# Graph-COM/SUREL_Plus

Measured on AMD Instinct MI355X. Metric: query-pairs/sec (sample+SpJoin), higher is better.
Workload: dtype int32; 1 GPU; cit2-like LP: N=2,927,963 avg-deg 20.7 power-law graph, M=200, --num_steps 4 (m=3 hops); ranks_seen=1, distinct_devices=1, rng=philox

## Files before the change

surel_plus_amd/csrc/sjoin.hip:

```cpp
#include "sjoin_f64pair.hpp"

namespace subgacc {


template <bool F64, int KV, typename Val>
__device__ __forceinline__ void emit_rows(const JoinArgs &a, int lane, const int32_t *own_ids, const Val *own_val,
                                          int64_t na, const int32_t *pids, const Val *pval, int nb, int64_t t0,
                                          int64_t o, int64_t segj, int k, int k2, uint32_t magic) {
    const int64_t t = t0 + lane;
    const bool live = t < na;
    int32_t id = 0;
    Val va = 0;
    if (live) {
        id = own_ids[t];
        va = own_val[t];
    }
    int lo = 0, hi = live ? nb : 0;
    SJ_HOOK_SEARCH_RANGE(lo, hi);
    while (lo < hi) {
        const int mid = (lo + hi) >> 1;
        if (pids[mid] < id) lo = mid + 1;
        else hi = mid;
    }
    const bool hit = live && lo < nb && pids[lo] == id;
// ... 65 lines not shown
        ra = jj < half ? src : tgt, rb = jj < half ? tgt : src;
        int64_t sb, sn;
        join_row(a, src, sb, sn);
        if (sn <= a.star_cap) return;
        if (lane == 0) atomicOr(&a.flags[1], 2);
    } else
        ra = a.own[j], rb = join_partner(a, j);
    join_row(a, ra, ab, na);
    join_row(a, rb, bb, nb64);
    if (nb64 > (STAGE ? (int64_t)a.max_len : (int64_t)0x7FFFFFFF)) {
        if (lane == 0) atomicOr(&a.flags[3], 1);
        return;
    }
    const int nb = (int)nb64;
    const Val *data = (const Val *)a.data;
    if (STAGE) {
        for (int r = lane; r < nb; r += kJoinThreads) {
            pids[r] = a.indices[bb + r];
            pval[r] = data[bb + r];
        }
        __syncthreads();
    } else {
        pids = const_cast<int32_t *>(a.indices + bb);
        pval = const_cast<Val *>(data + bb);
    }
    const int64_t o = a.seg[j];
    const int k = a.k, k2 = 2 * k;
    const uint32_t magic = k2 > 0 ? ((1u << 20) + (uint32_t)k2 - 1u) / (uint32_t)k2 : 0u;
    for (int64_t t0 = 0; t0 < na; t0 += kWave)
        emit_rows<F64, KV, Val>(a, lane, a.indices + ab, data + ab, na, pids, pval, nb, t0, o, j, k, k2, magic);
}


template <int KV, int NT, bool K64, bool TAB = false>
__global__ __launch_bounds__(NT) void sjoin_keypair_kernel(const JoinArgs a, uint32_t pb, uint32_t pairs) {
    extern __shared__ __align__(16) unsigned char lds_raw[];
    static_assert(!(K64 && TAB), "a table row number is 32 bits");
    using Key = typename std::conditional<K64, unsigned long long, uint32_t>::type;
    constexpr int NW = NT / kWave;
    const bool xl = TAB && a.slot_id != nullptr;
    auto sfptr = [&](Key v) -> Key {
        if (!TAB) return v;
        return xl ? (Key)(a.slot_id[(int32_t)v] + 1) : (Key)((int32_t)v + a.val_add);
    };
    const int ML = a.max_len;
    Key *valT = (Key *)lds_raw;
    Key *pk = valT + ML;
    int32_t *idsT = (int32_t *)(pk + ML);
    const int kc = KV > 0 ? KV : a.k, w = 2 * kc;
    const int tid = threadIdx.x, lane = tid & (kWave - 1);
    const int wave = __builtin_amdgcn_readfirstlane(tid / kWave);
    const size_t stage_off = ((size_t)ML * (2 * sizeof(Key) + 4) + 15) & ~(size_t)15;
    float *stage = (float *)(lds_raw + stage_off) + wave * (kWave * w + 4);

    SJ_HOOK_PAIR_ENTRY();
    if (a.sized_here && (a.flags[3] & 64)) return;
    const uint32_t wg = (uint32_t)(blockIdx.x & (kXcds - 1)) * (gridDim.x / kXcds) + (blockIdx.x / kXcds);
    uint32_t p = wg, part = 0;
    if (a.split > 1) {
        p = wg / (uint32_t)a.split;
        part = wg - p * (uint32_t)a.split;
    }
    if (p >= pairs) return;
    uint32_t blk = 0, off = p;
    if (pb != pairs) {
        blk = p / pb;
        off = p - blk * pb;
// ... 139 lines not shown
        }
#pragma unroll
        for (int u = 0; u < kRegTrips; ++u) {
            sgot[u] = 0;
            if (u < trips) {
                const int32_t f = idsT[b[u]];
                const Key g = valT[b[u]];
                const bool hit = (wave + u * NW) * kWave + lane < ns && n == 1 && f == sid[u];
                if (hit) pk[b[u]] = skey[u], sgot[u] = g;
            }
        }
    }
    for (int c = wave + kRegTrips * NW; c < chunksS; c += NW) {
        const int t0 = c * kWave;
        const bool live = t0 + lane < ns;
        int32_t id = 0;
        Key key = 0;
        if (live) {
            id = stream_load(&a.indices[sb + t0 + lane]);
            key = sfptr(stream_load(&keys[sb + t0 + lane]));
        }
        int bx = 0, n = nt;
        SJ_HOOK_SEARCH_RANGE(bx, n);
        while (n > 1) {
            const int h = n >> 1;
            bx = idsT[bx + h] <= id ? bx + h : bx;
            n -= h;
        }
        const int32_t f = idsT[bx];
        const Key g = valT[bx];
        const bool hit = live && n == 1 && f == id;
        if (hit) pk[bx] = key;
        if (whole || (uint32_t)(c / NW) % (uint32_t)a.split == part)
            emit_key_span<KV, K64, TAB, Key>(a, lane, live, key, hit ? g : (Key)0, ns - t0 < kWave ? ns - t0 : kWave, oS + t0, jS, kc, q, stage);
    }
    __syncthreads();
#pragma unroll
    for (int u = 0; u < kRegTrips; ++u) {
        const int c = wave + u * NW, t0 = c * kWave;
        if (c < chunksS && (whole || (uint32_t)u % (uint32_t)a.split == part))
            emit_key_span<KV, K64, TAB, Key>(a, lane, t0 + lane < ns, skey[u], sgot[u], ns - t0 < kWave ? ns - t0 : kWave, oS + t0, jS, kc, q, stage);
    }
    const int rot = (NW - chunksS % NW) % NW;
    for (int c = (wave + rot) % NW + (int)part * NW; c < chunksT; c += a.split * NW) {
        const int t0 = c * kWave;
        const bool live = t0 + lane < nt;
        const int i = live ? t0 + lane : t0;
        emit_key_span<KV, K64, TAB, Key>(a, lane, live, valT[i], pk[i], nt - t0 < kWave ? nt - t0 : kWave, oT + t0, jT, kc, q, stage);
    }
}


template <int NT>
__global__ __launch_bounds__(NT) void sjoin_f64pair_kernel(const JoinArgs a, uint32_t pb, uint32_t pairs) {
    extern __shared__ __align__(16) unsigned char lds_raw[];
    constexpr int NW = NT / kWave;
    const int ML = a.max_len;
    double *valT = (double *)lds_raw;
    double *pv = valT + ML;
    int32_t *idsT = (int32_t *)(pv + ML);
    const int tid = threadIdx.x;
    const int wave = __builtin_amdgcn_readfirstlane(tid / kWave);

    SJ_HOOK_PAIR_ENTRY();
    if (a.sized_here && (a.flags[3] & 64)) return;
    F64Pair p;
    float2 *xz = reinterpret_cast<float2 *>(a.out_xz);
    int64_t *segid = a.out_segid;
    int32_t *flags = a.flags;
    const auto span_s = [xz, segid, &p](int t, bool emit, double v, double got) {
        if (emit) {
            float2 o;
            o.x = (float)v, o.y = (float)((got + 1.0) - 1.0);
            stream_store(xz + p.oS + t, o);
            if (segid) __builtin_nontemporal_store(p.jS, segid + p.oS + t);
        }
    };
    if (!f64pair_stage<NT, true>(a, pb, pairs, ML, valT, pv, idsT, p, span_s, [flags, tid]() {
            if (tid == 0) atomicOr(&flags[3], 1);
        }))
        return;
    __syncthreads();
    const int chunksS = (p.ns + kWave - 1) / kWave, chunksT = (p.nt + kWave - 1) / kWave;
    const int rot = (NW - chunksS % NW) % NW;
    for (int c = (wave + rot) % NW + (int)p.part * NW; c < chunksT; c += a.split * NW) {
        const int t = c * kWave + (tid & (kWave - 1));
        if (t < p.nt) {
            float2 o;
            o.x = (float)valT[t], o.y = (float)((pv[t] + 1.0) - 1.0);
            stream_store(xz + p.oT + t, o);
            if (a.out_segid) __builtin_nontemporal_store(p.jT, a.out_segid + p.oT + t);
        }
    }
}

template <int KV, int NT, int MODE>
__global__ __launch_bounds__(NT) void sjoin_star_kernel(const JoinArgs a, uint32_t P, uint32_t K, uint32_t chunk, uint32_t chunks) {
    extern __shared__ __align__(16) unsigned char lds_raw[];
    constexpr bool F64 = MODE == 2, TAB = MODE == 1;
    using Val = typename std::conditional<F64, double, uint32_t>::type;
    constexpr int NW = NT / kWave;
    const int cap = a.star_cap;
    Val *valA = (Val *)lds_raw;
    Val *pa = valA + cap;
    int32_t *idsA = (int32_t *)(pa + cap);
    const int kc = F64 ? 1 : (KV > 0 ? KV : a.k), w = 2 * kc;
    const int tid = threadIdx.x, lane = tid & (kWave - 1);
    const int wave = __builtin_amdgcn_readfirstlane(tid / kWave);
    const size_t stage_off = ((size_t)cap * (2 * sizeof(Val) + 4) + 15) & ~(size_t)15;
    float *stage = (float *)(lds_raw + stage_off) + wave * (kWave * w + 4);

    if (a.sized_here && (a.flags[3] & 64)) return;
    if (blockIdx.x == 0 && tid == 0) atomicOr(&a.flags[1], 1);
    const uint32_t wg = (uint32_t)(blockIdx.x & (kXcds - 1)) * (gridDim.x / kXcds) + (blockIdx.x / kXcds);
    const uint32_t p = wg / chunks, part = wg - p * chunks;
    if (p >= P) return;
    const uint32_t t_beg = part * chunk, t_end = t_beg + chunk < K ? t_beg + chunk : K;
    if (t_beg >= t_end) return;
    int64_t ab, na64;
    join_row(a, a.own[p], ab, na64);
    if (na64 > cap) {
        if (na64 > a.max_len && tid == 0) atomicOr(&a.flags[3], 1);
        return;
    }
    const int na = (int)na64;
    const Val *vals = (const Val *)a.data;
    for (int r = tid; r < na; r += NT) {
        idsA[r] = a.indices[ab + r];
        valA[r] = vals[ab + r];
// ... 6 lines not shown
    const int64_t half = (int64_t)P * K;
    __syncthreads();
    for (uint32_t t = t_beg; t < t_end; ++t) {
        const int64_t j = (int64_t)p * K + t, j2 = half + j;
        int64_t bb, nb64;
        join_row(a, a.partner[j], bb, nb64);
        const int nb = (int)nb64;
        const int64_t oA = a.seg[j], oB = a.seg[j2];
        const int chunksB = (nb + kWave - 1) / kWave;
        for (int c = wave; c < chunksB; c += NW) {
            const int t0 = c * kWave;
            const bool live = t0 + lane < nb;
            int32_t id = 0;
            Val v = 0;
            if (live) {
                id = stream_load(&a.indices[bb + t0 + lane]);
                v = stream_load(&vals[bb + t0 + lane]);
            }
            int bx;
            const bool hit = sorted_find(idsA, na, id, live, bx);
            Val g = 0;
            if (hit) {
                pa[bx] = v;
                g = valA[bx];
            }
            if constexpr (F64) {
                if (live) {
                    float2 o;
                    o.x = (float)v, o.y = (float)((g + 1.0) - 1.0);
                    stream_store(xz + oB + t0 + lane, o);
                    if (a.out_segid) __builtin_nontemporal_store(j2, a.out_segid + oB + t0 + lane);
                }
            } else
                emit_key_span<KV, false, TAB, uint32_t>(a, lane, live, v, g, nb - t0 < kWave ? nb - t0 : kWave, oB + t0, j2, kc, q, stage);
        }
        __syncthreads();
        const int rot = (NW - chunksB % NW) % NW;
        for (int c = (wave + rot) % NW; c < chunksA; c += NW) {
            const int t0 = c * kWave;
            const bool live = t0 + lane < na;
            const int i = live ? t0 + lane : t0;
            const Val v = valA[i], g = pa[i];
            if (live) pa[i] = 0;
            if constexpr (F64) {
                if (live) {
                    float2 o;
                    o.x = (float)v, o.y = (float)((g + 1.0) - 1.0);
                    stream_store(xz + oA + i, o);
                    if (a.out_segid) __builtin_nontemporal_store(j, a.out_segid + oA + i);
                }
            } else
                emit_key_span<KV, false, TAB, uint32_t>(a, lane, live, v, g, na - t0 < kWave ? na - t0 : kWave, oA + t0, j, kc, q, stage);
        }
        __syncthreads();
    }
}

}

using namespace subgacc;


static int launch_table_pairs(JoinArgs &a, int64_t S, int64_t pair_block, bool vec4, void *stream, const char *who) {
    const int k = a.out_xz ? a.k : 1;
    const size_t lds = (size_t)a.max_len * 12 + key_stage_bytes(kPairEmit / kWave, k);
    SG_REQUIRE(lds <= (size_t)kLdsBytes, SUBGACC_ERR_LDS, "%s: rows of %d members do not fit LDS", who, (int)a.max_len);
    a.split = pair_split(S / 2);
    int64_t grid;
    if (int rc = grid_of(S / 2 * a.split, who, grid)) return rc;
    void (*kernel)(JoinArgs, uint32_t, uint32_t);
    if (vec4) kernel = sjoin_keypair_kernel<4, kPairEmit, false, true>;
    else if (a.out_xz && a.k == 3) kernel = sjoin_keypair_kernel<3, kPairEmit, false, true>;
    else if (a.out_xz && a.k == 5) kernel = sjoin_keypair_kernel<5, kPairEmit, false, true>;
    else kernel = sjoin_keypair_kernel<0, kPairEmit, false, true>;
    return launch(kernel, grid, kPairEmit, lds, (hipStream_t)stream, a, (uint32_t)pair_block, (uint32_t)(S / 2));
}

static int key_args(JoinArgs &a, int32_t num_walks, int32_t num_steps, const char *who, bool wide) {
    const int shift = subgacc_key_shift(num_walks, num_steps);
    if (shift < 0) return shift;
    SG_REQUIRE(num_steps * shift + 1 <= (wide ? 63 : 31) && num_steps + 1 <= 16, SUBGACC_ERR_KEYWIDTH,
               "%s: LP keys of %d steps x %d bits do not fit %d bits", who, num_steps, shift, wide ? 64 : 32);
    a.k = num_steps + 1;
    a.key_M = num_walks, a.key_m = num_steps, a.key_shift = shift;
    return SUBGACC_OK;
}

static int launch_key_join(JoinArgs &a, int32_t num_walks, int32_t num_steps, int64_t S, int64_t pair_block, void *stream,
                           const char *who, bool wide = false) {
    const int rc = key_args(a, num_walks, num_steps, who, wide);
    if (rc != SUBGACC_OK) return rc;
    const int nt = (a.max_len > 512 && pair_split(S / 2) == 1 && (a.k == 4 || (wide && a.k == 5))) ? 256 : kPairEmit;
    const size_t lds = (size_t)a.max_len * (wide ? 20 : 12) + key_stage_bytes(nt / kWave, a.k);
    SG_REQUIRE(lds <= (size_t)kLdsBytes, SUBGACC_ERR_LDS, "%s: rows of %d members do not fit LDS", who, (int)a.max_len);
    a.split = pair_split(S / 2);
    int64_t grid;
    if (int rc = grid_of(S / 2 * a.split, who, grid)) return rc;
    void (*kernel)(JoinArgs, uint32_t, uint32_t);
    int threads = kPairEmit;
    if (wide) {
        if (a.k == 5 && nt == 256) kernel = sjoin_keypair_kernel<5, 256, true>, threads = 256;
        else if (a.k == 5) kernel = sjoin_keypair_kernel<5, kPairEmit, true>;
        else kernel = sjoin_keypair_kernel<0, kPairEmit, true>;
    } else if (a.k == 4 && nt == 256) kernel = sjoin_keypair_kernel<4, 256, false>, threads = 256;
    else if (a.k == 4) kernel = sjoin_keypair_kernel<4, kPairEmit, false>;
    else if (a.k == 3) kernel = sjoin_keypair_kernel<3, kPairEmit, false>;
    else if (a.k == 5) kernel = sjoin_keypair_kernel<5, kPairEmit, false>;
    else kernel = sjoin_keypair_kernel<0, kPairEmit, false>;
    return launch(kernel, grid, threads, lds, (hipStream_t)stream, a, (uint32_t)pair_block, (uint32_t)(S / 2));
}

static int launch_f64_pairs(JoinArgs &a, int64_t S, int64_t pair_block, void *stream) {
    const size_t flds = (size_t)a.max_len * 20 + 16;
    SG_REQUIRE(flds <= (size_t)kLdsBytes, SUBGACC_ERR_LDS, "sjoin_fill: float rows of %d members do not fit LDS", (int)a.max_len);
    a.split = pair_split(S / 2);
    int64_t grid;
    if (int rc = grid_of(S / 2 * a.split, "sjoin_fill", grid)) return rc;
    const uint32_t pairs = (uint32_t)(S / 2), pb32 = (uint32_t)pair_block;
    hipStream_t s = (hipStream_t)stream;
    if (a.max_len <= 2 * kWave) return launch(sjoin_f64pair_kernel<kWave>, grid, kWave, flds, s, a, pb32, pairs);
    return launch(sjoin_f64pair_kernel<kPairEmit>, grid, kPairEmit, flds, s, a, pb32, pairs);
}

static int launch_segments(JoinArgs &a, bool f64, bool vec4, void *stream) {
    size_t lds = (size_t)a.max_len * (f64 ? 12 : 8);
    const bool staged = lds <= (size_t)kLdsBytes;
    if (!staged) lds = 0;
    int64_t grid;
    if (int rc = grid_of(a.S, "sjoin_fill", grid)) return rc;
    void (*kernel)(JoinArgs);
    if (!staged) {
        if (f64) kernel = sjoin_fill_kernel<true, 0, false>;
        else if (vec4) kernel = sjoin_fill_kernel<false, 4, false>;
        else kernel = sjoin_fill_kernel<false, 0, false>;
    } else if (f64) kernel = sjoin_fill_kernel<true, 0>;
    else if (vec4) kernel = sjoin_fill_kernel<false, 4>;
    else kernel = sjoin_fill_kernel<false, 0>;
    return launch(kernel, grid, kJoinThreads, lds, (hipStream_t)stream, a);
}

#ifndef SJ_STAR_GROUPS
#define SJ_STAR_GROUPS 8192
#endif
constexpr int64_t kStarGroups = SJ_STAR_GROUPS;
static int launch_star(JoinArgs &a, int mode, bool vec4, bool packed, int64_t K, void *stream) {
    const int64_t S = a.S, P = S / (2 * K);
    SG_REQUIRE(S / 2 < (1ll << 31), SUBGACC_ERR_BADARG, "sjoin_fill_v2: the star option (OPT_STAR) joins fewer than 2^31 pairs, not %lld", (long long)(S / 2));
    const bool f64 = mode == 2;
    const int nt = f64 && a.max_len <= 2 * kWave ? kWave : kPairEmit;
    const size_t per = f64 ? 20 : 12, stage = f64 ? 16 : key_stage_bytes(nt / kWave, a.k);
    const size_t room = (size_t)kLdsBytes - stage - 16;
    int64_t cap = a.max_len;
    if ((size_t)cap * per > room) cap = (int64_t)(room / per);
    SG_REQUIRE(cap == a.max_len || (packed && mode != 0), SUBGACC_ERR_LDS, "sjoin_fill_v2: rows of %d members do not fit LDS",
               (int)a.max_len);
    a.star_k = K, a.star_cap = (int32_t)cap;
    int64_t chunks = ceil_div(kStarGroups, P);
    if (chunks > K) chunks = K;
    const int64_t chunk = ceil_div(K, chunks);
    chunks = ceil_div(K, chunk);
    int64_t grid;
    if (int rc = grid_of(P * chunks, "sjoin_fill_v2", grid)) return rc;
    const size_t lds = (((size_t)cap * per + 15) & ~(size_t)15) + stage;
    void (*kernel)(JoinArgs, uint32_t, uint32_t, uint32_t, uint32_t);
    if (f64 && nt == kWave) kernel = sjoin_star_kernel<0, kWave, 2>;
    else if (f64) kernel = sjoin_star_kernel<0, kPairEmit, 2>;
    else if (mode == 1 && vec4) kernel = sjoin_star_kernel<4, kPairEmit, 1>;
    else if (mode == 1 && a.k == 3) kernel = sjoin_star_kernel<3, kPairEmit, 1>;
    else if (mode == 1 && a.k == 5) kernel = sjoin_star_kernel<5, kPairEmit, 1>;
    else if (mode == 1) kernel = sjoin_star_kernel<0, kPairEmit, 1>;
    else if (a.k == 4) kernel = sjoin_star_kernel<4, kPairEmit, 0>;
    else if (a.k == 3) kernel = sjoin_star_kernel<3, kPairEmit, 0>;
    else if (a.k == 5) kernel = sjoin_star_kernel<5, kPairEmit, 0>;
    else kernel = sjoin_star_kernel<0, kPairEmit, 0>;
    if (int rc = launch(kernel, grid, nt, lds, (hipStream_t)stream, a, (uint32_t)P, (uint32_t)K, (uint32_t)chunk, (uint32_t)chunks))
        return rc;
    if (cap < a.max_len) return launch_segments(a, f64, vec4, stream);
    return SUBGACC_OK;
}

extern "C" int subgacc_sjoin_fill_v2(const subgacc_join_desc *d, void *stream) {
    RowLayout layout;
    if (int rc = decode_desc("sjoin_fill_v2", d, false, layout)) return rc;
    const bool packed = layout == RowLayout::Packed, strided = layout == RowLayout::Strided;
    SG_REQUIRE((d->options & ~(SUBGACC_JOIN_OPT_SIZES | SUBGACC_JOIN_OPT_STAR)) == 0, SUBGACC_ERR_BADARG,
               "sjoin_fill_v2: unknown option bits %d", (int)d->options);
    SG_REQUIRE(d->form >= SUBGACC_JOIN_ROWS && d->form <= SUBGACC_JOIN_PAIRS, SUBGACC_ERR_BADARG, "sjoin_fill_v2: unknown form %d", (int)d->form);
    SG_REQUIRE(d->payload_kind >= SUBGACC_JOIN_SFPTR && d->payload_kind <= SUBGACC_JOIN_KEY64, SUBGACC_ERR_BADARG,
               "sjoin_fill_v2: unknown payload kind %d", (int)d->payload_kind);
    const int kind = d->payload_kind;
    const bool f64 = kind == SUBGACC_JOIN_F64, keyed = kind == SUBGACC_JOIN_KEY32 || kind == SUBGACC_JOIN_KEY64;
    const bool sized = (d->options & SUBGACC_JOIN_OPT_SIZES) != 0;
    const bool sizes_only = sized && !d->out_xz && !d->out_idx;
    const bool star = (d->options & SUBGACC_JOIN_OPT_STAR) != 0;
    const int64_t *seg = sized ? d->out_seg : d->seg;
    const int64_t S = d->S, pb = d->pair_block;
    SG_REQUIRE(!sized || d->form == SUBGACC_JOIN_ROWS, SUBGACC_ERR_BADARG, "sjoin_fill_v2: OPT_SIZES goes with the row form");
    if (star) {
        SG_REQUIRE(d->form == SUBGACC_JOIN_ROWS, SUBGACC_ERR_BADARG, "sjoin_fill_v2: the star option (OPT_STAR) goes with the row form (not the count or pair form)");
        SG_REQUIRE(!strided, SUBGACC_ERR_BADARG, "sjoin_fill_v2: the star option (OPT_STAR) joins packed or headed rows, not strided rows");
        SG_REQUIRE(kind != SUBGACC_JOIN_KEY64, SUBGACC_ERR_BADARG, "sjoin_fill_v2: the star option (OPT_STAR) does not join 64-bit keys (KEY64)");
        SG_REQUIRE(pb > 0, SUBGACC_ERR_BADARG, "sjoin_fill_v2: the star option (OPT_STAR) needs pair_block = K > 0 targets per source (pair_block = %lld)",
                   (long long)pb);
// ... 81 lines not shown
```

surel_plus_amd/csrc/sjoin.hpp:

```cpp
#pragma once
#include <cstdlib>
#include <type_traits>
#include "common.hpp"

namespace subgacc {

constexpr int kJoinThreads = 64;
constexpr int kPairThreads = 256;
#ifndef SJ_PAIR_THREADS
#define SJ_PAIR_THREADS 128
#endif
constexpr int kPairEmit = SJ_PAIR_THREADS;
constexpr int kMeanThreads = kPairEmit;
constexpr int kMeanCap = 1024;

struct JoinArgs {
    const int64_t *indptr;
    const int32_t *indices;
    const void *data;
    const int64_t *own, *partner, *seg;
    int64_t S;
    int64_t n_rows;
    const float *table;
    int64_t table_rows;
// ... 116 lines not shown
            sid[u] = 0, sval[u] = 0;
            if (r < ns) sid[u] = stream_load(&a.indices[sb + r]), sval[u] = stream_load(&data[sb + r]);
        }
    }
    __device__ __forceinline__ void get(const JoinArgs &a, int64_t sb, int r0, int r, int32_t &id, int32_t &value) const {
        const int u = r0 / kPairThreads;
        const int32_t i0 = sid[0], i1 = sid[1], v0 = sval[0], v1 = sval[1];
        if (u < kTrips) {
            id = u == 0 ? i0 : i1;
            value = u == 0 ? v0 : v1;
        } else {
            id = stream_load(&a.indices[sb + r]);
            value = stream_load(&((const int32_t *)a.data)[sb + r]);
        }
    }
};

struct KeyQuot {
    float fm, rcp;
    bool divide;
};
__device__ __forceinline__ float lp_quotient(uint32_t c, const KeyQuot &q) {
    const float a = (float)c;
    if (q.divide) return a / q.fm;
    const float q0 = a * q.rcp;
    return __fmaf_rn(__fmaf_rn(-q.fm, q0, a), q.rcp, q0);
}
template <bool K64>
__device__ __forceinline__ float key_field(typename std::conditional<K64, unsigned long long, uint32_t>::type key, int c, int m, int shift,
                                           const KeyQuot &q) {
    if (c == 0) return (float)(uint32_t)((key >> (m * shift)) & 1u);
    return lp_quotient((uint32_t)(key >> ((m - c) * shift)) & ((1u << shift) - 1u), q);
}

template <int KV, bool K64, bool TAB, typename Key>
__device__ __forceinline__ void emit_key_span(const JoinArgs &a, int lane, bool live, Key ka, Key kb, int nrows, int64_t row0, int64_t segj,
                                              int kc, const KeyQuot &q, float *stage) {
    const int w = 2 * kc, m = kc - 1, shift = a.key_shift;
    if (TAB) {
        if (a.out_idx && live) {
            int2 v;
            v.x = (int32_t)ka, v.y = (int32_t)kb;
            stream_store(reinterpret_cast<int2 *>(a.out_idx) + row0 + lane, v);
        }
        if (!a.out_xz) {
            if (a.out_segid && live) __builtin_nontemporal_store(segj, a.out_segid + row0 + lane);
            return;
        }
        if (live && ((uint64_t)ka >= (uint64_t)a.table_rows || (uint64_t)kb >= (uint64_t)a.table_rows)) {
            atomicOr(&a.flags[3], 2);
            ka = kb = 0;
        }
    }
    float *dst = a.out_xz + row0 * w;
    const int mis = (int)(((uintptr_t)dst >> 2) & 3);
    const int head = (4 - mis) & 3;
    if (live) {
        float *mine = stage + mis + lane * w;
        if (TAB && KV == 4) {
            const float4 fa = reinterpret_cast<const float4 *>(a.table)[(uint32_t)ka], fb = reinterpret_cast<const float4 *>(a.table)[(uint32_t)kb];
            mine[0] = fa.x, mine[1] = fa.y, mine[2] = fa.z, mine[3] = fa.w;
            mine[4] = fb.x, mine[5] = fb.y, mine[6] = fb.z, mine[7] = fb.w;
        } else if (TAB && KV > 0) {
            const float *ta = a.table + (int64_t)(uint32_t)ka * KV, *tb = a.table + (int64_t)(uint32_t)kb * KV;
            float f[2 * (KV > 0 ? KV : 1)];
#pragma unroll
            for (int c = 0; c < KV; ++c) f[c] = ta[c], f[KV + c] = tb[c];
#pragma unroll
            for (int c = 0; c < 2 * KV; ++c) mine[c] = f[c];
        } else if (TAB) {
            const float *ta = a.table + (int64_t)(uint32_t)ka * kc, *tb = a.table + (int64_t)(uint32_t)kb * kc;
            for (int c = 0; c < kc; ++c) {
                mine[c] = ta[c];
                mine[kc + c] = tb[c];
            }
        } else if (KV > 0) {
            float f[2 * (KV > 0 ? KV : 1)];
#pragma unroll
            for (int c = 0; c < KV; ++c) {
                f[c] = key_field<K64>(ka, c, m, shift, q);
                f[KV + c] = key_field<K64>(kb, c, m, shift, q);
            }
#pragma unroll
            for (int c = 0; c < 2 * KV; ++c) mine[c] = f[c];
        } else
            for (int c = 0; c < kc; ++c) {
                mine[c] = key_field<K64>(ka, c, m, shift, q);
                mine[kc + c] = key_field<K64>(kb, c, m, shift, q);
            }
    }
    __builtin_amdgcn_fence(__ATOMIC_RELEASE, "wavefront");
    __builtin_amdgcn_wave_barrier();
    __builtin_amdgcn_fence(__ATOMIC_ACQUIRE, "wavefront");
    const int total = nrows * w;
    const int nbody = SJ_HOOK_SPAN_STORES(total > head ? (total - head) >> 2 : 0);
    const int ntail = total > head ? (total - head) & 3 : 0;
    const float *src = stage + mis;
    const float4 *src4 = reinterpret_cast<const float4 *>(src + head);
    float4 *dst4 = reinterpret_cast<float4 *>(dst + head);
    if (mis | ntail) {
        const int i = kWave - 1 - lane;
        if (i < head && i < total) __builtin_nontemporal_store(src[i], dst + i);
        const int t2 = kWave - 4 - lane, at = head + 4 * nbody;
        if (t2 >= 0 && t2 < ntail) __builtin_nontemporal_store(src[at + t2], dst + at + t2);
    }
    if (KV > 0) {
#pragma unroll
        for (int qd = 0; qd < (KV + 1) / 2; ++qd) {
            const int f = lane + qd * kWave;
            if (f < nbody) stream_store(dst4 + f, src4[f]);
        }
    } else
        for (int f = lane; f < nbody; f += kWave) stream_store(dst4 + f, src4[f]);
    __builtin_amdgcn_fence(__ATOMIC_RELEASE, "wavefront");
    __builtin_amdgcn_wave_barrier();
    if (a.out_segid && live) __builtin_nontemporal_store(segj, a.out_segid + row0 + lane);
}

static inline int pair_split(int64_t pairs) {
#ifdef SG_DEV_JOIN_SPLIT
    return SG_DEV_JOIN_SPLIT;
#endif
    int sp = 1;
    while (sp < 2 && pairs * sp * 2 <= 4096) sp *= 2;
    return sp;
}
// ... 69 lines not shown
```

surel_plus_amd/csrc/sjoin_packed.hip:

```cpp
#include "sjoin.hpp"
#include "packed_rows.hpp"
#include "waveops.hpp"
#include "../../include/subgacc_packed.h"

namespace subgacc {

template <int KV, int NT, int RT>
__global__ __launch_bounds__(NT) void sjoin_packpair_kernel(const JoinArgs a, const int32_t *__restrict__ nesc, int cb, int fb, uint32_t pb,
                                                            uint32_t pairs) {
    extern __shared__ __align__(16) unsigned char lds_raw[];
    using Key = uint32_t;
    constexpr int NW = NT / kWave, MH = KV - 1, kRegTrips = RT, kChunks = kRegTrips * NW;
    constexpr int kEsc = kWave;
    static_assert(kChunks <= 16, "the chunk counts of S and T share one wave scan: 16 lanes each");
    static_assert((2 * kEsc + 32) * 4 <= NW * (kWave * 2 * KV + 4) * 4, "the escape staging lies inside the per-wave staging areas");
    const int ML = a.max_len;
    Key *valT = (Key *)lds_raw;
    Key *pk = valT + ML;
    int32_t *idsT = (int32_t *)(pk + ML);
    constexpr int kc = KV, w = 2 * kc;
    const int tid = threadIdx.x, lane = tid & (kWave - 1);
    const int wave = __builtin_amdgcn_readfirstlane(tid / kWave);
    const size_t stage_off = ((size_t)ML * 12 + 15) & ~(size_t)15;
    float *stage0 = (float *)(lds_raw + stage_off);
    float *stage = stage0 + wave * (kWave * w + 4);
    Key *escS = (Key *)stage0, *escT = escS + kEsc;
    int32_t *ccnt = (int32_t *)(escT + kEsc);
    const uint32_t ones = (1u << cb) - 1u;
    const int shift = a.key_shift;

    const uint32_t wg = (uint32_t)(blockIdx.x & (kXcds - 1)) * (gridDim.x / kXcds) + (blockIdx.x / kXcds);
    uint32_t p = wg, part = 0;
    if (a.split > 1) {
        p = wg / (uint32_t)a.split;
        part = wg - p * (uint32_t)a.split;
    }
    if (p >= pairs) return;
    uint32_t blk = 0, off = p;
    if (pb != pairs) {
        blk = p / pb;
// ... 30 lines not shown
        if (tid == 0) atomicOr(&a.flags[3], 1);
        return;
    }
    const bool swap = na > nb;
    const int ns = swap ? nb : na, nt = swap ? na : nb;
    const int64_t sb = swap ? bb : ab, tb = swap ? ab : bb;
    const int64_t oS = swap ? oB : oA, oT = swap ? oA : oB, jS = swap ? j2 : j, jT = swap ? j : j2;
    const int neS = swap ? neB : neA, neT = swap ? neA : neB;
    const int capS = neS < 0 ? 0 : (neS > ML ? ML : neS), capT = neT < 0 ? 0 : (neT > ML ? ML : neT);
    uint32_t sw[kRegTrips], tw[kRegTrips];
    sw[0] = swap ? wB0 : wA0, tw[0] = swap ? wA0 : wB0;
#pragma unroll
    for (int u = 1; u < kRegTrips; ++u) {
        const int r = tid + u * NT;
        sw[u] = 0, tw[u] = 0;
        if (u * NT < nt) {
            sw[u] = stream_load(&words[sb + (r < ns ? r : 0)]);
            tw[u] = stream_load(&words[tb + (r < nt ? r : 0)]);
        }
    }
#pragma unroll
    for (int u = 0; u < kRegTrips; ++u) {
        const int r = tid + u * NT;
        sw[u] = r < ns ? sw[u] : 0u, tw[u] = r < nt ? tw[u] : 0u;
    }
    if (wave == 0) {
        escS[lane] = swap ? eB0 : eA0;
        escT[lane] = swap ? eA0 : eB0;
    }
    unsigned long long balS[kRegTrips], balT[kRegTrips];
#pragma unroll
    for (int u = 0; u < kRegTrips; ++u) {
        const int r = tid + u * NT, c = u * NW + wave;
        balS[u] = __ballot(r < ns && (sw[u] & ones) == ones);
        balT[u] = __ballot(r < nt && (tw[u] & ones) == ones);
        if (lane == 0) ccnt[c] = __popcll(balS[u]), ccnt[16 + c] = __popcll(balT[u]);
        if (r < nt) {
            idsT[r] = (int32_t)(tw[u] >> cb);
            pk[r] = 0;
        }
    }
    __syncthreads();
    int32_t sid[kRegTrips];
    Key skey[kRegTrips], sgot[kRegTrips];
    {
        const int cv = (lane < 32 && (lane & 15) < kChunks) ? ccnt[lane] : 0;
        const int incl = wave_scan_add_i32_incl(cv);
        const int totS = __builtin_amdgcn_readlane(incl, 15), totT = __builtin_amdgcn_readlane(incl, 31) - totS;
        if (tid == 0 && (totS != neS || totT != neT)) atomicOr(&a.flags[3], 2);
        const unsigned long long below = (1ull << lane) - 1ull;
        auto key_of = [&](uint32_t word, bool live, int rank, const Key *staged, int cap, int64_t rowb) -> Key {
            if (!live) return 0;
            const uint32_t code = word & ones;
            if (code != ones) return unpack_code<MH>(code, shift, fb);
            if (rank >= cap) {
                atomicOr(&a.flags[3], 2);
                return 0;
            }
            return rank < kEsc ? staged[rank] : stream_load(&escs[rowb + rank]);
        };
#pragma unroll
        for (int u = 0; u < kRegTrips; ++u) {
            const int r = tid + u * NT, c = u * NW + wave;
            const int baseS = c ? __builtin_amdgcn_readlane(incl, c - 1) : 0;
            const int baseT = __builtin_amdgcn_readlane(incl, 15 + c) - totS;
            sid[u] = r < ns ? (int32_t)(sw[u] >> cb) : 0;
            skey[u] = key_of(sw[u], r < ns, baseS + __popcll(balS[u] & below), escS, capS, sb);
            if (r < nt) valT[r] = key_of(tw[u], true, baseT + __popcll(balT[u] & below), escT, capT, tb);
        }
    }
    __syncthreads();

    const int chunksS = (ns + kWave - 1) / kWave, chunksT = (nt + kWave - 1) / kWave;
    const bool whole = a.split == 1;
    {
        int b[kRegTrips];
#pragma unroll
        for (int u = 0; u < kRegTrips; ++u) b[u] = 0;
        int n = nt;
        const int trips = (chunksS - wave + NW - 1) / NW;
        while (n > 1) {
            const int h = n >> 1;
#pragma unroll
            for (int u = 0; u < kRegTrips; ++u)
                if (u < trips) b[u] = idsT[b[u] + h] <= sid[u] ? b[u] + h : b[u];
            n -= h;
        }
#pragma unroll
        for (int u = 0; u < kRegTrips; ++u) {
            sgot[u] = 0;
            if (u < trips) {
                const int32_t f = idsT[b[u]];
                const Key g = valT[b[u]];
                const bool hit = (wave + u * NW) * kWave + lane < ns && n == 1 && f == sid[u];
                if (hit) pk[b[u]] = skey[u], sgot[u] = g;
            }
        }
    }
    __syncthreads();
#pragma unroll
    for (int u = 0; u < kRegTrips; ++u) {
        const int c = wave + u * NW, t0 = c * kWave;
        if (c < chunksS && (whole || (uint32_t)u % (uint32_t)a.split == part))
            emit_key_span<KV, false, false, Key>(a, lane, t0 + lane < ns, skey[u], sgot[u], ns - t0 < kWave ? ns - t0 : kWave, oS + t0, jS, kc, q, stage);
    }
    const int rot = (NW - chunksS % NW) % NW;
    for (int c = (wave + rot) % NW + (int)part * NW; c < chunksT; c += a.split * NW) {
        const int t0 = c * kWave;
        const bool live = t0 + lane < nt;
        const int i = live ? t0 + lane : t0;
        emit_key_span<KV, false, false, Key>(a, lane, live, valT[i], pk[i], nt - t0 < kWave ? nt - t0 : kWave, oT + t0, jT, kc, q, stage);
    }
}

__global__ __launch_bounds__(kWave) void unpack_packed_rows_kernel(const uint32_t *__restrict__ words, const uint32_t *__restrict__ escs,
                                                                   const int32_t *__restrict__ nsize, const int32_t *__restrict__ nesc,
                                                                   int64_t n, int32_t pitch, int cb, int fb, int m, int shift,
                                                                   int32_t *__restrict__ out_ids, int32_t *__restrict__ out_keys,
                                                                   int32_t *__restrict__ flags) {
    const int64_t r = blockIdx.x;
    if (r >= n) return;
    const int lane = threadIdx.x;
    int ns = nsize[r];
    if (ns > pitch) ns = pitch;
    int cap = nesc[r];
    cap = cap < 0 ? 0 : (cap > pitch ? pitch : cap);
    const int64_t rowb = r * (int64_t)pitch;
    const uint32_t ones = (1u << cb) - 1u;
    const unsigned long long below = (1ull << lane) - 1ull;
    int base = 0;
    for (int x0 = 0; x0 < ns; x0 += kWave) {
        const int x = x0 + lane;
        const bool live = x < ns;
        const uint32_t word = live ? words[rowb + x] : 0u;
        const bool esc = live && (word & ones) == ones;
        const unsigned long long bal = __ballot(esc);
        uint32_t key = 0;
        if (esc) {
            const int rank = base + __popcll(bal & below);
            if (rank < cap) key = escs[rowb + rank];
            else atomicOr(&flags[3], 2);
        } else if (live)
            key = unpack_code(word & ones, m, shift, fb);
        if (live) {
// ... 17 lines not shown
    return SUBGACC_OK;
}

extern "C" int subgacc_sjoin_fill_packed(const subgacc_join_desc *d, const int32_t *nesc, int64_t num_nodes, void *stream) {
    const char *who = "sjoin_fill_packed";
    RowLayout layout;
    if (int rc = decode_desc(who, d, false, layout)) return rc;
    SG_REQUIRE(d->form == SUBGACC_JOIN_ROWS && d->options == 0 && d->payload_kind == SUBGACC_JOIN_KEY32 && layout == RowLayout::Strided,
               SUBGACC_ERR_BADARG, "%s: the row form over strided rows of 32-bit keys (payload_kind KEY32, row_len), no option bits", who);
    const int64_t S = d->S, pb = d->pair_block;
    SG_REQUIRE(pb > 0 && S % (2 * pb) == 0, SUBGACC_ERR_BADARG, "%s: a mirrored list (pair_block > 0, S a multiple of 2*pair_block)", who);
    SG_REQUIRE(!d->out_idx && !d->out_counts && !d->out_pairs && !d->out_mult && !d->out_cnt && !d->out_seg, SUBGACC_ERR_BADARG,
               "%s: writes out_xz (and out_segid) only", who);
    const int shift = subgacc_key_shift(d->num_walks, d->num_steps);
    if (shift < 0) return shift;
    SG_REQUIRE(d->num_steps * shift + 1 <= 31, SUBGACC_ERR_KEYWIDTH, "%s: LP keys of %d steps x %d bits do not fit 32 bits", who,
               (int)d->num_steps, shift);
    PackFmt f;
    if (int rc = packed_format(who, num_nodes, d->num_steps, f)) return rc;
    if (S == 0) return SUBGACC_OK;
    SG_REQUIRE(d->flags && d->ids && d->payload && nesc && d->own && d->seg && d->out_xz, SUBGACC_ERR_BADARG,
               "%s: null argument (flags / ids / payload / nesc / own / seg / out_xz)", who);
    JoinArgs a = join_args(d, layout);
    a.seg = d->seg, a.out_xz = d->out_xz, a.out_segid = d->out_segid;
    a.k = d->num_steps + 1, a.key_M = d->num_walks, a.key_m = d->num_steps, a.key_shift = shift;
    const int nt = a.max_len > 640 ? 256 : kPairEmit, rt = a.max_len > 512 && a.max_len <= 640 ? 5 : 4;
    SG_REQUIRE(a.max_len <= rt * nt, SUBGACC_ERR_LDS, "%s: rows of %d members (the packed join holds %d)", who, (int)a.max_len, rt * nt);
    const size_t lds = (size_t)a.max_len * 12 + key_stage_bytes(nt / kWave, a.k);
    SG_REQUIRE(lds <= (size_t)kLdsBytes, SUBGACC_ERR_LDS, "%s: rows of %d members do not fit LDS", who, (int)a.max_len);
    a.split = pair_split(S / 2);
    int64_t grid;
    if (int rc = grid_of(S / 2 * a.split, who, grid)) return rc;
    void (*kernel)(JoinArgs, const int32_t *, int, int, uint32_t, uint32_t);
    if (nt == 256) kernel = a.k == 3 ? sjoin_packpair_kernel<3, 256, 4> : a.k == 4 ? sjoin_packpair_kernel<4, 256, 4> : sjoin_packpair_kernel<5, 256, 4>;
    else if (rt == 5) kernel = a.k == 3 ? sjoin_packpair_kernel<3, kPairEmit, 5> : a.k == 4 ? sjoin_packpair_kernel<4, kPairEmit, 5> : sjoin_packpair_kernel<5, kPairEmit, 5>;
    else kernel = a.k == 3 ? sjoin_packpair_kernel<3, kPairEmit, 4> : a.k == 4 ? sjoin_packpair_kernel<4, kPairEmit, 4> : sjoin_packpair_kernel<5, kPairEmit, 4>;
    return launch(kernel, grid, nt, lds, (hipStream_t)stream, a, nesc, (int)f.cb, (int)f.fb, (uint32_t)pb, (uint32_t)(S / 2));
}

extern "C" int subgacc_unpack_packed_rows(const int32_t *row_words, const int32_t *row_esc, const int32_t *nsize, const int32_t *nesc, int64_t n,
                                          int32_t row_pitch, int64_t num_nodes, int32_t num_walks, int32_t num_steps, int32_t *out_ids,
                                          int32_t *out_keys, int32_t *flags, void *stream) {
    const char *who = "unpack_packed_rows";
    SG_REQUIRE(n >= 0 && row_pitch > 0, SUBGACC_ERR_BADARG, "%s: bad arguments (n = %lld, row_pitch = %d)", who, (long long)n, (int)row_pitch);
    const int shift = subgacc_key_shift(num_walks, num_steps);
    if (shift < 0) return shift;
    SG_REQUIRE(num_steps * shift + 1 <= 31, SUBGACC_ERR_KEYWIDTH, "%s: LP keys of %d steps x %d bits do not fit 32 bits", who, (int)num_steps, shift);
    PackFmt f;
    if (int rc = packed_format(who, num_nodes, num_steps, f)) return rc;
    if (n == 0) return SUBGACC_OK;
    SG_REQUIRE(row_words && row_esc && nsize && nesc && out_ids && out_keys && flags, SUBGACC_ERR_BADARG, "%s: null argument", who);
    SG_REQUIRE(n < (1ll << 31), SUBGACC_ERR_BADARG, "%s: too many rows in one call", who);
    return launch(unpack_packed_rows_kernel, n, kWave, 0, (hipStream_t)stream, (const uint32_t *)row_words, (const uint32_t *)row_esc, nsize, nesc, n,
                  row_pitch, (int)f.cb, (int)f.fb, (int)num_steps, shift, out_ids, out_keys, flags);
}
```

Before: 63.35 million query-pairs/s.

## Add aligned float4 span stores, exact-divide path, branchless escape decode in packed join

Adds a template flag to the key-span emitter. When k is even and the output is 16-byte aligned, each lane writes its whole row into LDS as float4 and the wave streams it out with full-width stores, skipping the misalignment head/tail logic. When num_walks is large, an exact division path replaces the reciprocal-refined quotient. The packed pair kernel also decodes escape codes branchlessly, loading global escapes only when a row actually needs them, and specialises the multi-trip binary search by trip count. These changes add more kernel instantiations and a different numeric path for large walk counts.

```diff
diff --git a/surel_plus_amd/csrc/sjoin.hip b/surel_plus_amd/csrc/sjoin.hip
--- a/surel_plus_amd/csrc/sjoin.hip
+++ b/surel_plus_amd/csrc/sjoin.hip
@@ -121,7 +121,7 @@
 }
 
 
-template <int KV, int NT, bool K64, bool TAB = false>
+template <int KV, int NT, bool K64, bool TAB = false, int F = 0>
 __global__ __launch_bounds__(NT) void sjoin_keypair_kernel(const JoinArgs a, uint32_t pb, uint32_t pairs) {
     extern __shared__ __align__(16) unsigned char lds_raw[];
     static_assert(!(K64 && TAB), "a table row number is 32 bits");
@@ -327,21 +327,21 @@
         const bool hit = live && n == 1 && f == id;
         if (hit) pk[bx] = key;
         if (whole || (uint32_t)(c / NW) % (uint32_t)a.split == part)
-            emit_key_span<KV, K64, TAB, Key>(a, lane, live, key, hit ? g : (Key)0, ns - t0 < kWave ? ns - t0 : kWave, oS + t0, jS, kc, q, stage);
+            emit_key_span<KV, K64, TAB, Key, F>(a, lane, live, key, hit ? g : (Key)0, ns - t0 < kWave ? ns - t0 : kWave, oS + t0, jS, kc, q, stage);
     }
     __syncthreads();
 #pragma unroll
     for (int u = 0; u < kRegTrips; ++u) {
         const int c = wave + u * NW, t0 = c * kWave;
         if (c < chunksS && (whole || (uint32_t)u % (uint32_t)a.split == part))
-            emit_key_span<KV, K64, TAB, Key>(a, lane, t0 + lane < ns, skey[u], sgot[u], ns - t0 < kWave ? ns - t0 : kWave, oS + t0, jS, kc, q, stage);
+            emit_key_span<KV, K64, TAB, Key, F>(a, lane, t0 + lane < ns, skey[u], sgot[u], ns - t0 < kWave ? ns - t0 : kWave, oS + t0, jS, kc, q, stage);
     }
     const int rot = (NW - chunksS % NW) % NW;
     for (int c = (wave + rot) % NW + (int)part * NW; c < chunksT; c += a.split * NW) {
         const int t0 = c * kWave;
         const bool live = t0 + lane < nt;
         const int i = live ? t0 + lane : t0;
-        emit_key_span<KV, K64, TAB, Key>(a, lane, live, valT[i], pk[i], nt - t0 < kWave ? nt - t0 : kWave, oT + t0, jT, kc, q, stage);
+        emit_key_span<KV, K64, TAB, Key, F>(a, lane, live, valT[i], pk[i], nt - t0 < kWave ? nt - t0 : kWave, oT + t0, jT, kc, q, stage);
     }
 }
 
@@ -389,7 +389,7 @@
     }
 }
 
-template <int KV, int NT, int MODE>
+template <int KV, int NT, int MODE, int F = 0>
 __global__ __launch_bounds__(NT) void sjoin_star_kernel(const JoinArgs a, uint32_t P, uint32_t K, uint32_t chunk, uint32_t chunks) {
     extern __shared__ __align__(16) unsigned char lds_raw[];
     constexpr bool F64 = MODE == 2, TAB = MODE == 1;
@@ -462,7 +462,7 @@
                     if (a.out_segid) __builtin_nontemporal_store(j2, a.out_segid + oB + t0 + lane);
                 }
             } else
-                emit_key_span<KV, false, TAB, uint32_t>(a, lane, live, v, g, nb - t0 < kWave ? nb - t0 : kWave, oB + t0, j2, kc, q, stage);
+                emit_key_span<KV, false, TAB, uint32_t, F>(a, lane, live, v, g, nb - t0 < kWave ? nb - t0 : kWave, oB + t0, j2, kc, q, stage);
         }
         __syncthreads();
         const int rot = (NW - chunksB % NW) % NW;
@@ -480,7 +480,7 @@
                     if (a.out_segid) __builtin_nontemporal_store(j, a.out_segid + oA + i);
                 }
             } else
-                emit_key_span<KV, false, TAB, uint32_t>(a, lane, live, v, g, na - t0 < kWave ? na - t0 : kWave, oA + t0, j, kc, q, stage);
+                emit_key_span<KV, false, TAB, uint32_t, F>(a, lane, live, v, g, na - t0 < kWave ? na - t0 : kWave, oA + t0, j, kc, q, stage);
         }
         __syncthreads();
     }
@@ -520,7 +520,9 @@
                            const char *who, bool wide = false) {
     const int rc = key_args(a, num_walks, num_steps, who, wide);
     if (rc != SUBGACC_OK) return rc;
-    const int nt = (a.max_len > 512 && pair_split(S / 2) == 1 && (a.k == 4 || (wide && a.k == 5))) ? 256 : kPairEmit;
+    const bool divide = (span_form(num_walks, 0, a.out_xz) & kSpanDivide) != 0;
+    const bool al4 = (span_form(num_walks, 4, a.out_xz) & kSpanAligned) != 0;
+    const int nt = (!divide && a.max_len > 512 && pair_split(S / 2) == 1 && (a.k == 4 || (wide && a.k == 5))) ? 256 : kPairEmit;
     const size_t lds = (size_t)a.max_len * (wide ? 20 : 12) + key_stage_bytes(nt / kWave, a.k);
     SG_REQUIRE(lds <= (size_t)kLdsBytes, SUBGACC_ERR_LDS, "%s: rows of %d members do not fit LDS", who, (int)a.max_len);
     a.split = pair_split(S / 2);
@@ -528,12 +530,14 @@
     if (int rc = grid_of(S / 2 * a.split, who, grid)) return rc;
     void (*kernel)(JoinArgs, uint32_t, uint32_t);
     int threads = kPairEmit;
-    if (wide) {
+    if (divide) kernel = wide ? sjoin_keypair_kernel<0, kPairEmit, true, false, kSpanDivide> : sjoin_keypair_kernel<0, kPairEmit, false, false, kSpanDivide>;
+    else if (wide) {
         if (a.k == 5 && nt == 256) kernel = sjoin_keypair_kernel<5, 256, true>, threads = 256;
         else if (a.k == 5) kernel = sjoin_keypair_kernel<5, kPairEmit, true>;
         else kernel = sjoin_keypair_kernel<0, kPairEmit, true>;
-    } else if (a.k == 4 && nt == 256) kernel = sjoin_keypair_kernel<4, 256, false>, threads = 256;
-    else if (a.k == 4) kernel = sjoin_keypair_kernel<4, kPairEmit, false>;
+    } else if (a.k == 4 && nt == 256)
+        kernel = al4 ? sjoin_keypair_kernel<4, 256, false, false, kSpanAligned> : sjoin_keypair_kernel<4, 256, false>, threads = 256;
+    else if (a.k == 4) kernel = al4 ? sjoin_keypair_kernel<4, kPairEmit, false, false, kSpanAligned> : sjoin_keypair_kernel<4, kPairEmit, false>;
     else if (a.k == 3) kernel = sjoin_keypair_kernel<3, kPairEmit, false>;
     else if (a.k == 5) kernel = sjoin_keypair_kernel<5, kPairEmit, false>;
     else kernel = sjoin_keypair_kernel<0, kPairEmit, false>;
@@ -599,6 +603,8 @@
     else if (mode == 1 && a.k == 3) kernel = sjoin_star_kernel<3, kPairEmit, 1>;
     else if (mode == 1 && a.k == 5) kernel = sjoin_star_kernel<5, kPairEmit, 1>;
     else if (mode == 1) kernel = sjoin_star_kernel<0, kPairEmit, 1>;
+    else if (span_form(a.key_M, 0, a.out_xz) & kSpanDivide) kernel = sjoin_star_kernel<0, kPairEmit, 0, kSpanDivide>;
+    else if (a.k == 4 && (span_form(a.key_M, 4, a.out_xz) & kSpanAligned)) kernel = sjoin_star_kernel<4, kPairEmit, 0, kSpanAligned>;
     else if (a.k == 4) kernel = sjoin_star_kernel<4, kPairEmit, 0>;
     else if (a.k == 3) kernel = sjoin_star_kernel<3, kPairEmit, 0>;
     else if (a.k == 5) kernel = sjoin_star_kernel<5, kPairEmit, 0>;
diff --git a/surel_plus_amd/csrc/sjoin.hpp b/surel_plus_amd/csrc/sjoin.hpp
--- a/surel_plus_amd/csrc/sjoin.hpp
+++ b/surel_plus_amd/csrc/sjoin.hpp
@@ -172,10 +172,30 @@
     if (c == 0) return (float)(uint32_t)((key >> (m * shift)) & 1u);
     return lp_quotient((uint32_t)(key >> ((m - c) * shift)) & ((1u << shift) - 1u), q);
 }
-
-template <int KV, bool K64, bool TAB, typename Key>
+template <bool DIV>
+__device__ __forceinline__ float lp_quotient(uint32_t c, const KeyQuot &q) {
+    const float a = (float)c;
+    if (DIV) return a / q.fm;
+    const float q0 = a * q.rcp;
+    return __fmaf_rn(__fmaf_rn(-q.fm, q0, a), q.rcp, q0);
+}
+template <bool K64, bool DIV>
+__device__ __forceinline__ float key_field(typename std::conditional<K64, unsigned long long, uint32_t>::type key, int c, int m, int shift,
+                                           const KeyQuot &q) {
+    if (c == 0) return (float)(uint32_t)((key >> (m * shift)) & 1u);
+    return lp_quotient<DIV>((uint32_t)(key >> ((m - c) * shift)) & ((1u << shift) - 1u), q);
+}
+
+constexpr int kSpanDivide = 1, kSpanAligned = 2;
+static inline int span_form(int32_t num_walks, int kv, const float *out_xz) {
+    return (num_walks >= 4096 ? kSpanDivide : 0) | (kv > 0 && kv % 2 == 0 && ((uintptr_t)out_xz & 15) == 0 ? kSpanAligned : 0);
+}
+
+template <int KV, bool K64, bool TAB, typename Key, int F = 0>
 __device__ __forceinline__ void emit_key_span(const JoinArgs &a, int lane, bool live, Key ka, Key kb, int nrows, int64_t row0, int64_t segj,
                                               int kc, const KeyQuot &q, float *stage) {
+    constexpr bool DIV = (F & kSpanDivide) != 0, AL = (F & kSpanAligned) != 0;
+    static_assert(!AL || (KV > 0 && KV % 2 == 0), "an aligned span is made of rows of whole 16-byte words");
     const int w = 2 * kc, m = kc - 1, shift = a.key_shift;
     if (TAB) {
         if (a.out_idx && live) {
@@ -193,7 +213,7 @@
         }
     }
     float *dst = a.out_xz + row0 * w;
-    const int mis = (int)(((uintptr_t)dst >> 2) & 3);
+    const int mis = AL ? 0 : (int)(((uintptr_t)dst >> 2) & 3);
     const int head = (4 - mis) & 3;
     if (live) {
         float *mine = stage + mis + lane * w;
@@ -214,24 +234,47 @@
                 mine[c] = ta[c];
                 mine[kc + c] = tb[c];
             }
+        } else if (AL) {
+            float4 *mine4 = reinterpret_cast<float4 *>(mine);
+#pragma unroll
+            for (int c4 = 0; c4 < 2 * KV; c4 += 4) {
+                float f[4];
+#pragma unroll
+                for (int i = 0; i < 4; ++i) f[i] = key_field<K64, DIV>(c4 + i < KV ? ka : kb, (c4 + i) % (KV > 0 ? KV : 1), m, shift, q);
+                mine4[c4 / 4] = make_float4(f[0], f[1], f[2], f[3]);
+            }
         } else if (KV > 0) {
             float f[2 * (KV > 0 ? KV : 1)];
 #pragma unroll
             for (int c = 0; c < KV; ++c) {
-                f[c] = key_field<K64>(ka, c, m, shift, q);
-                f[KV + c] = key_field<K64>(kb, c, m, shift, q);
+                f[c] = key_field<K64, DIV>(ka, c, m, shift, q);
+                f[KV + c] = key_field<K64, DIV>(kb, c, m, shift, q);
             }
 #pragma unroll
             for (int c = 0; c < 2 * KV; ++c) mine[c] = f[c];
         } else
             for (int c = 0; c < kc; ++c) {
-                mine[c] = key_field<K64>(ka, c, m, shift, q);
-                mine[kc + c] = key_field<K64>(kb, c, m, shift, q);
+                mine[c] = key_field<K64, DIV>(ka, c, m, shift, q);
+                mine[kc + c] = key_field<K64, DIV>(kb, c, m, shift, q);
             }
     }
     __builtin_amdgcn_fence(__ATOMIC_RELEASE, "wavefront");
     __builtin_amdgcn_wave_barrier();
     __builtin_amdgcn_fence(__ATOMIC_ACQUIRE, "wavefront");
+    if constexpr (AL) {
+        const int nbody = SJ_HOOK_SPAN_STORES(nrows * (KV / 2));
+        const float4 *src4 = reinterpret_cast<const float4 *>(stage);
+        float4 *dst4 = reinterpret_cast<float4 *>(a.out_xz) + row0 * (KV / 2);
+#pragma unroll
+        for (int qd = 0; qd < KV / 2; ++qd) {
+            const int f = lane + qd * kWave;
+            if (f < nbody) stream_store(dst4 + f, src4[f]);
+        }
+        __builtin_amdgcn_fence(__ATOMIC_RELEASE, "wavefront");
+        __builtin_amdgcn_wave_barrier();
+        if (a.out_segid && live) __builtin_nontemporal_store(segj, a.out_segid + row0 + lane);
+        return;
+    }
     const int total = nrows * w;
     const int nbody = SJ_HOOK_SPAN_STORES(total > head ? (total - head) >> 2 : 0);
     const int ntail = total > head ? (total - head) & 3 : 0;
diff --git a/surel_plus_amd/csrc/sjoin_packed.hip b/surel_plus_amd/csrc/sjoin_packed.hip
--- a/surel_plus_amd/csrc/sjoin_packed.hip
+++ b/surel_plus_amd/csrc/sjoin_packed.hip
@@ -5,7 +5,35 @@
 
 namespace subgacc {
 
-template <int KV, int NT, int RT>
+template <int TR, int NW, int RT, typename Key>
+__device__ __forceinline__ void search_trips(int trips, const int32_t *idsT, const Key *valT, Key *pk, int nt, int ns, int wave, int lane,
+                                             const int32_t (&sid)[RT], const Key (&skey)[RT], Key (&sgot)[RT]) {
+    if constexpr (TR > 0) {
+        if (trips < TR) {
+            search_trips<TR - 1, NW, RT, Key>(trips, idsT, valT, pk, nt, ns, wave, lane, sid, skey, sgot);
+            return;
+        }
+        int b[TR];
+#pragma unroll
+        for (int u = 0; u < TR; ++u) b[u] = 0;
+        int n = nt;
+        while (n > 1) {
+            const int h = n >> 1;
+#pragma unroll
+            for (int u = 0; u < TR; ++u) b[u] = idsT[b[u] + h] <= sid[u] ? b[u] + h : b[u];
+            n -= h;
+        }
+#pragma unroll
+        for (int u = 0; u < TR; ++u) {
+            const int32_t f = idsT[b[u]];
+            const Key g = valT[b[u]];
+            const bool hit = (wave + u * NW) * kWave + lane < ns && n == 1 && f == sid[u];
+            if (hit) pk[b[u]] = skey[u], sgot[u] = g;
+        }
+    }
+}
+
+template <int KV, int NT, int RT, int F = 0>
 __global__ __launch_bounds__(NT) void sjoin_packpair_kernel(const JoinArgs a, const int32_t *__restrict__ nesc, int cb, int fb, uint32_t pb,
                                                             uint32_t pairs) {
     extern __shared__ __align__(16) unsigned char lds_raw[];
@@ -102,8 +130,8 @@
 #pragma unroll
     for (int u = 0; u < kRegTrips; ++u) {
         const int r = tid + u * NT, c = u * NW + wave;
-        balS[u] = __ballot(r < ns && (sw[u] & ones) == ones);
-        balT[u] = __ballot(r < nt && (tw[u] & ones) == ones);
+        balS[u] = __ballot((sw[u] & ones) == ones);
+        balT[u] = __ballot((tw[u] & ones) == ones);
         if (lane == 0) ccnt[c] = __popcll(balS[u]), ccnt[16 + c] = __popcll(balT[u]);
         if (r < nt) {
             idsT[r] = (int32_t)(tw[u] >> cb);
@@ -119,24 +147,29 @@
         const int totS = __builtin_amdgcn_readlane(incl, 15), totT = __builtin_amdgcn_readlane(incl, 31) - totS;
         if (tid == 0 && (totS != neS || totT != neT)) atomicOr(&a.flags[3], 2);
         const unsigned long long below = (1ull << lane) - 1ull;
-        auto key_of = [&](uint32_t word, bool live, int rank, const Key *staged, int cap, int64_t rowb) -> Key {
-            if (!live) return 0;
-            const uint32_t code = word & ones;
-            if (code != ones) return unpack_code<MH>(code, shift, fb);
-            if (rank >= cap) {
-                atomicOr(&a.flags[3], 2);
-                return 0;
-            }
-            return rank < kEsc ? staged[rank] : stream_load(&escs[rowb + rank]);
-        };
+        const bool far = (totS > kEsc && capS > kEsc) || (totT > kEsc && capT > kEsc), bad = totS > capS || totT > capT;
 #pragma unroll
         for (int u = 0; u < kRegTrips; ++u) {
             const int r = tid + u * NT, c = u * NW + wave;
             const int baseS = c ? __builtin_amdgcn_readlane(incl, c - 1) : 0;
             const int baseT = __builtin_amdgcn_readlane(incl, 15 + c) - totS;
-            sid[u] = r < ns ? (int32_t)(sw[u] >> cb) : 0;
-            skey[u] = key_of(sw[u], r < ns, baseS + __popcll(balS[u] & below), escS, capS, sb);
-            if (r < nt) valT[r] = key_of(tw[u], true, baseT + __popcll(balT[u] & below), escT, capT, tb);
+            const uint32_t codeS = sw[u] & ones, codeT = tw[u] & ones;
+            const bool isS = codeS == ones, isT = codeT == ones;
+            const int rankS = baseS + __popcll(balS[u] & below), rankT = baseT + __popcll(balT[u] & below);
+            Key eS = escS[rankS < kEsc ? rankS : kEsc - 1], eT = escT[rankT < kEsc ? rankT : kEsc - 1];
+            if (far) {
+                if (isS && rankS >= kEsc && rankS < capS) eS = stream_load(&escs[sb + rankS]);
+                if (isT && rankT >= kEsc && rankT < capT) eT = stream_load(&escs[tb + rankT]);
+            }
+            if (bad) {
+                if ((isS && rankS >= capS) || (isT && rankT >= capT)) atomicOr(&a.flags[3], 2);
+            }
+            const Key uS = unpack_code<MH>(codeS, shift, fb), uT = unpack_code<MH>(codeT, shift, fb);
+            const Key kS = isS ? (rankS < capS ? eS : 0u) : uS;
+            const Key kT = isT ? (rankT < capT ? eT : 0u) : uT;
+            sid[u] = (int32_t)(sw[u] >> cb);
+            skey[u] = kS;
+            if (r < nt) valT[r] = kT;
         }
     }
     __syncthreads();
@@ -144,42 +177,24 @@
     const int chunksS = (ns + kWave - 1) / kWave, chunksT = (nt + kWave - 1) / kWave;
     const bool whole = a.split == 1;
     {
-        int b[kRegTrips];
-#pragma unroll
-        for (int u = 0; u < kRegTrips; ++u) b[u] = 0;
-        int n = nt;
         const int trips = (chunksS - wave + NW - 1) / NW;
-        while (n > 1) {
-            const int h = n >> 1;
-#pragma unroll
-            for (int u = 0; u < kRegTrips; ++u)
-                if (u < trips) b[u] = idsT[b[u] + h] <= sid[u] ? b[u] + h : b[u];
-            n -= h;
-        }
-#pragma unroll
-        for (int u = 0; u < kRegTrips; ++u) {
-            sgot[u] = 0;
-            if (u < trips) {
-                const int32_t f = idsT[b[u]];
-                const Key g = valT[b[u]];
-                const bool hit = (wave + u * NW) * kWave + lane < ns && n == 1 && f == sid[u];
-                if (hit) pk[b[u]] = skey[u], sgot[u] = g;
-            }
-        }
+#pragma unroll
+        for (int u = 0; u < kRegTrips; ++u) sgot[u] = 0;
+        search_trips<kRegTrips, NW, kRegTrips>(trips, idsT, valT, pk, nt, ns, wave, lane, sid, skey, sgot);
     }
     __syncthreads();
 #pragma unroll
     for (int u = 0; u < kRegTrips; ++u) {
         const int c = wave + u * NW, t0 = c * kWave;
         if (c < chunksS && (whole || (uint32_t)u % (uint32_t)a.split == part))
-            emit_key_span<KV, false, false, Key>(a, lane, t0 + lane < ns, skey[u], sgot[u], ns - t0 < kWave ? ns - t0 : kWave, oS + t0, jS, kc, q, stage);
+            emit_key_span<KV, false, false, Key, F>(a, lane, t0 + lane < ns, skey[u], sgot[u], ns - t0 < kWave ? ns - t0 : kWave, oS + t0, jS, kc, q, stage);
     }
     const int rot = (NW - chunksS % NW) % NW;
     for (int c = (wave + rot) % NW + (int)part * NW; c < chunksT; c += a.split * NW) {
         const int t0 = c * kWave;
         const bool live = t0 + lane < nt;
         const int i = live ? t0 + lane : t0;
-        emit_key_span<KV, false, false, Key>(a, lane, live, valT[i], pk[i], nt - t0 < kWave ? nt - t0 : kWave, oT + t0, jT, kc, q, stage);
+        emit_key_span<KV, false, false, Key, F>(a, lane, live, valT[i], pk[i], nt - t0 < kWave ? nt - t0 : kWave, oT + t0, jT, kc, q, stage);
     }
 }
 
@@ -263,9 +278,16 @@
     int64_t grid;
     if (int rc = grid_of(S / 2 * a.split, who, grid)) return rc;
     void (*kernel)(JoinArgs, const int32_t *, int, int, uint32_t, uint32_t);
-    if (nt == 256) kernel = a.k == 3 ? sjoin_packpair_kernel<3, 256, 4> : a.k == 4 ? sjoin_packpair_kernel<4, 256, 4> : sjoin_packpair_kernel<5, 256, 4>;
-    else if (rt == 5) kernel = a.k == 3 ? sjoin_packpair_kernel<3, kPairEmit, 5> : a.k == 4 ? sjoin_packpair_kernel<4, kPairEmit, 5> : sjoin_packpair_kernel<5, kPairEmit, 5>;
-    else kernel = a.k == 3 ? sjoin_packpair_kernel<3, kPairEmit, 4> : a.k == 4 ? sjoin_packpair_kernel<4, kPairEmit, 4> : sjoin_packpair_kernel<5, kPairEmit, 4>;
+    const int form = span_form(d->num_walks, a.k, a.out_xz);
+    SG_REQUIRE(!(form & kSpanDivide) || a.k == 3, SUBGACC_ERR_KEYWIDTH, "%s: num_walks = %d with %d steps", who, (int)d->num_walks, (int)d->num_steps);
+#define SG_PACKPAIR(NT_, RT_)                                                                                                   \
+    (a.k == 3 ? ((form & kSpanDivide) ? sjoin_packpair_kernel<3, NT_, RT_, kSpanDivide> : sjoin_packpair_kernel<3, NT_, RT_>)  \
+     : a.k == 4 ? ((form & kSpanAligned) ? sjoin_packpair_kernel<4, NT_, RT_, kSpanAligned> : sjoin_packpair_kernel<4, NT_, RT_>) \
+                : sjoin_packpair_kernel<5, NT_, RT_>)
+    if (nt == 256) kernel = SG_PACKPAIR(256, 4);
+    else if (rt == 5) kernel = SG_PACKPAIR(kPairEmit, 5);
+    else kernel = SG_PACKPAIR(kPairEmit, 4);
+#undef SG_PACKPAIR
     return launch(kernel, grid, nt, lds, (hipStream_t)stream, a, nesc, (int)f.cb, (int)f.fb, (uint32_t)pb, (uint32_t)(S / 2));
 }
 
```

New measurement: 62.74 million query-pairs/s. About the same (-1.0%).
